# KrishnaswamyLab/MELD

Measured on AMD Instinct MI355X. Metric: cells/sec through MELD.fit_transform (kNN+Chebyshev), higher is better.
Workload: dtype f64

## Files before the change

### meld_amd/csrc/frame.hip

```cpp
#include "common.hpp"

namespace meld {

constexpr int FR_ROWS = 64;
constexpr int FR_DMAX = 64;

__global__ __launch_bounds__(256) void cov_sample_kernel(const double* __restrict__ X, int64_t n_s, int64_t stride, int d,
                                                         const double* __restrict__ mean, double* __restrict__ out) {
  __shared__ double sx[FR_ROWS][FR_DMAX + 1];
  const int tid = threadIdx.x;
  const int64_t s0 = (int64_t)blockIdx.x * FR_ROWS;
  const int cnt = (int)min((int64_t)FR_ROWS, n_s - s0);
  for (int u = tid; u < FR_ROWS * d; u += 256) {
    const int r = u / d, k = u - r * d;
    sx[r][k] = r < cnt ? X[(s0 + r) * stride * d + k] - mean[k] : 0.0;
  }
  __syncthreads();
  for (int p = tid; p < d * d; p += 256) {
    const int i = p / d, j = p - i * d;
    if (j < i) continue;
    double acc = 0.0;
    for (int r = 0; r < FR_ROWS; ++r) acc = fma(sx[r][i], sx[r][j], acc);
    atomicAdd(out + p, acc);
  }
}

typedef double f64x8 __attribute__((ext_vector_type(8)));
typedef const __attribute__((address_space(4))) f64x8* const_f64x8_ptr;
constexpr int FR_LD = FR_DMAX + 1;
constexpr int FR_NQ = FR_ROWS * FR_DMAX / 256;
constexpr int FR_CPG = FR_DMAX / 4;
__global__ __launch_bounds__(256) void rotate_rows_kernel(const double* __restrict__ X, int64_t N, int d, const double* __restrict__ mean,
                                                          const double* __restrict__ At, double* __restrict__ out, int64_t tiles_per_wg) {
  __shared__ double sx[FR_ROWS][FR_LD];
  const int tid = threadIdx.x, lane = tid & 63;
  const int w = __builtin_amdgcn_readfirstlane(tid >> 6);
  const int cpg = (d + 3) >> 2;
  const int j0 = w * cpg;
  const int k8n = (d + 7) >> 3;
  const double mk = (lane < d) ? mean[lane] : 0.0;
  const int64_t n_tiles = (N + FR_ROWS - 1) / FR_ROWS;
  const int64_t t_begin = (int64_t)blockIdx.x * tiles_per_wg, t_end = min(n_tiles, t_begin + tiles_per_wg);
  double xv[FR_NQ];
  auto fetch = [&](int64_t t) __attribute__((always_inline)) {
    const int64_t row0 = t * FR_ROWS;
#pragma unroll
    for (int q = 0; q < FR_NQ; ++q) {
      const int u = tid + 256 * q, rr = u >> 6, k = u & 63;
      xv[q] = (t < t_end && row0 + rr < N && k < d) ? X[(row0 + rr) * d + k] : mk;
    }
  };
  fetch(t_begin);
  for (int64_t t = t_begin; t < t_end; ++t) {
    const int64_t row0 = t * FR_ROWS;
    const int cnt = (int)min((int64_t)FR_ROWS, N - row0);
    __syncthreads();
#pragma unroll
    for (int q = 0; q < FR_NQ; ++q) {
      const int u = tid + 256 * q, rr = u >> 6, k = u & 63;
      sx[rr][k] = xv[q] - mk;
    }
    fetch(t + 1);
    __syncthreads();
    double xr[FR_DMAX];
#pragma unroll
    for (int k = 0; k < FR_DMAX; ++k) xr[k] = sx[lane][k];
    double res[FR_CPG];
#pragma unroll
    for (int c4 = 0; c4 < FR_CPG; c4 += 4) {
      double acc[4] = {0.0, 0.0, 0.0, 0.0};
      if (c4 < cpg) {
        const_f64x8_ptr arow[4];
#pragma unroll
        for (int i = 0; i < 4; ++i)
          arow[i] = (const_f64x8_ptr)(uintptr_t)(At + (size_t)min(j0 + c4 + i, d - 1) * FR_DMAX);
#pragma unroll
        for (int k8 = 0; k8 < FR_DMAX / 8; ++k8) {
          if (k8 < k8n) {
            f64x8 av[4];
#pragma unroll
            for (int i = 0; i < 4; ++i) av[i] = arow[i][k8];
#pragma unroll
            for (int e = 0; e < 8; ++e)
#pragma unroll
              for (int i = 0; i < 4; ++i) acc[i] = fma(xr[8 * k8 + e], av[i][e], acc[i]);
          }
        }
      }
#pragma unroll
      for (int i = 0; i < 4; ++i) res[c4 + i] = acc[i];
    }
    __syncthreads();
#pragma unroll
    for (int c = 0; c < FR_CPG; ++c)
      if (c < cpg && j0 + c < d) sx[lane][j0 + c] = res[c];
    __syncthreads();
#pragma unroll
    for (int q = 0; q < FR_NQ; ++q) {
      const int u = tid + 256 * q, rr = u >> 6, k = u & 63;
      if (rr < cnt && k < d) out[(row0 + rr) * d + k] = sx[rr][k];
    }
  }
}

}

using namespace meld;

extern "C" int meld_frame_max_dims(void) { return FR_DMAX; }

extern "C" int meld_cov_sample_f64(const double* X, int64_t N, int d, const double* mean, int64_t stride, double* cov, meld_stream_t stream) {
  MELD_CHECK_ARG(X && mean && cov && N > 0 && d > 0 && d <= FR_DMAX && stride >= 1, "meld_cov_sample_f64: bad arguments (d <= %d)", FR_DMAX);
  const int64_t n_s = (N + stride - 1) / stride;
  hipLaunchKernelGGL(cov_sample_kernel, dim3((unsigned)ceil_div(n_s, FR_ROWS)), dim3(256), 0, S(stream), X, n_s, stride, d, mean, cov);
  MELD_LAUNCH_CHECK("cov_sample_kernel");
  return MELD_OK;
}

extern "C" int meld_rotate_rows_f64(const double* X, int64_t N, int d, const double* mean, const double* At, double* out, meld_stream_t stream) {
  MELD_CHECK_ARG(X && mean && At && out && N > 0 && d > 0 && d <= FR_DMAX && X != out, "meld_rotate_rows_f64: bad arguments (d <= %d)", FR_DMAX);
  const int64_t tiles = ceil_div(N, FR_ROWS);
  const int64_t per = ceil_div(tiles, (int64_t)1024);
  hipLaunchKernelGGL(rotate_rows_kernel, dim3((unsigned)ceil_div(tiles, per)), dim3(256), 0, S(stream), X, N, d, mean, At, out, per);
  MELD_LAUNCH_CHECK("rotate_rows_kernel");
  return MELD_OK;
}
```

Before: 28.52 million.

## Rework rotate_rows kernel with templated column count, LDS-staged At and 2-row register tiling

The row-rotation kernel becomes a template on columns-per-wave, specialised at runtime from d. The At matrix and the mean are staged in dynamic LDS, each lane computes two rows per tile, the tile grows to 128 rows, and global loads and stores use contiguous flat indexing with a d-dependent padded LDS stride. The aim is to cut wasted work for d<64, reduce scalar global reads of At, and coalesce I/O. In exchange it adds sixteen instantiations, larger LDS use, and a hipFuncSetAttribute path. That path's size formula differs from the launch size, and the d&7 branch adds dummy fma no-ops.

New measurement: 28.44 million. About the same (-0.3%).

```diff
diff --git a/meld_amd/csrc/frame.hip b/meld_amd/csrc/frame.hip
--- a/meld_amd/csrc/frame.hip
+++ b/meld_amd/csrc/frame.hip
@@ -25,82 +25,105 @@
   }
 }
 
-typedef double f64x8 __attribute__((ext_vector_type(8)));
-typedef const __attribute__((address_space(4))) f64x8* const_f64x8_ptr;
-constexpr int FR_LD = FR_DMAX + 1;
-constexpr int FR_NQ = FR_ROWS * FR_DMAX / 256;
-constexpr int FR_CPG = FR_DMAX / 4;
-__global__ __launch_bounds__(256) void rotate_rows_kernel(const double* __restrict__ X, int64_t N, int d, const double* __restrict__ mean,
-                                                          const double* __restrict__ At, double* __restrict__ out, int64_t tiles_per_wg) {
-  __shared__ double sx[FR_ROWS][FR_LD];
+constexpr int RT_ROWS = 128;
+__host__ __device__ inline int rt_ld(int d) { return d + ((2 - d) & 3); }
+template <int C>
+__global__ __launch_bounds__(256, C <= 13 ? 2 : 1) void rotate_rows_kernel(const double* __restrict__ X, int64_t N, int d, const double* __restrict__ mean,
+                                                             const double* __restrict__ At, double* __restrict__ out, int64_t tiles_per_wg) {
+  extern __shared__ __attribute__((aligned(16))) double rt_lds[];
+  constexpr int NQ = 2 * C;
   const int tid = threadIdx.x, lane = tid & 63;
   const int w = __builtin_amdgcn_readfirstlane(tid >> 6);
-  const int cpg = (d + 3) >> 2;
-  const int j0 = w * cpg;
-  const int k8n = (d + 7) >> 3;
-  const double mk = (lane < d) ? mean[lane] : 0.0;
-  const int64_t n_tiles = (N + FR_ROWS - 1) / FR_ROWS;
+  const int ld = rt_ld(d), np = (d + 1) >> 1;
+  double* sx = rt_lds;
+  double* sa = sx + RT_ROWS * ld;
+  double* sm = sa + np * 4 * C * 2;
+  for (int u = tid; u < np * 4 * C * 2; u += 256) {
+    const int e = u & 1, j = (u >> 1) % (4 * C), k = 2 * ((u >> 1) / (4 * C)) + e;
+    sa[u] = (j < d && k < FR_DMAX) ? At[(size_t)j * FR_DMAX + k] : 0.0;
+  }
+  if (tid < d) sm[tid] = mean[tid];
+  for (int u = tid; u < RT_ROWS * (ld - d); u += 256) sx[(u / (ld - d)) * ld + d + u % (ld - d)] = 0.0;
+  const int r0 = tid / d, k0 = tid - r0 * d, dr = 256 / d, dk = 256 - dr * d;
+  const int64_t n_tiles = (N + RT_ROWS - 1) / RT_ROWS;
   const int64_t t_begin = (int64_t)blockIdx.x * tiles_per_wg, t_end = min(n_tiles, t_begin + tiles_per_wg);
-  double xv[FR_NQ];
+  double xv[NQ];
   auto fetch = [&](int64_t t) __attribute__((always_inline)) {
-    const int64_t row0 = t * FR_ROWS;
+    const int64_t row0 = t * RT_ROWS;
+    if (t >= t_end) return;
+    const int last = (int)min((int64_t)RT_ROWS, N - row0) * d - 1;
+    const double* src = X + row0 * d;
 #pragma unroll
-    for (int q = 0; q < FR_NQ; ++q) {
-      const int u = tid + 256 * q, rr = u >> 6, k = u & 63;
-      xv[q] = (t < t_end && row0 + rr < N && k < d) ? X[(row0 + rr) * d + k] : mk;
-    }
+    for (int q = 0; q < NQ; ++q) xv[q] = src[min(tid + 256 * q, last)];
   };
   fetch(t_begin);
   for (int64_t t = t_begin; t < t_end; ++t) {
-    const int64_t row0 = t * FR_ROWS;
-    const int cnt = (int)min((int64_t)FR_ROWS, N - row0);
+    const int64_t row0 = t * RT_ROWS;
+    const int n_el = (int)min((int64_t)RT_ROWS, N - row0) * d;
     __syncthreads();
+    {
+      int r = r0, k = k0;
 #pragma unroll
-    for (int q = 0; q < FR_NQ; ++q) {
-      const int u = tid + 256 * q, rr = u >> 6, k = u & 63;
-      sx[rr][k] = xv[q] - mk;
+      for (int q = 0; q < NQ; ++q) {
+        if (tid + 256 * q < RT_ROWS * d) sx[r * ld + k] = xv[q] - sm[k];
+        r += dr, k += dk;
+        if (k >= d) k -= d, ++r;
+      }
     }
     fetch(t + 1);
     __syncthreads();
-    double xr[FR_DMAX];
+    double acc[2][C];
 #pragma unroll
-    for (int k = 0; k < FR_DMAX; ++k) xr[k] = sx[lane][k];
-    double res[FR_CPG];
+    for (int c = 0; c < C; ++c) acc[0][c] = acc[1][c] = 0.0;
+    {
+      const double2* xa = (const double2*)(sx + lane * ld);
+      const double2* xb = (const double2*)(sx + (lane + 64) * ld);
+      const double2* ap = (const double2*)sa + w * C;
+#pragma unroll 1
+      for (int p = 0; p < np; ++p, ap += 4 * C) {
+        const double2 a = xa[p], b = xb[p];
+        double2 av[C];
 #pragma unroll
-    for (int c4 = 0; c4 < FR_CPG; c4 += 4) {
-      double acc[4] = {0.0, 0.0, 0.0, 0.0};
-      if (c4 < cpg) {
-        const_f64x8_ptr arow[4];
+        for (int c = 0; c < C; ++c) av[c] = ap[c];
 #pragma unroll
-        for (int i = 0; i < 4; ++i)
-          arow[i] = (const_f64x8_ptr)(uintptr_t)(At + (size_t)min(j0 + c4 + i, d - 1) * FR_DMAX);
+        for (int c = 0; c < C; ++c) acc[0][c] = fma(a.x, av[c].x, acc[0][c]), acc[1][c] = fma(b.x, av[c].x, acc[1][c]);
 #pragma unroll
-        for (int k8 = 0; k8 < FR_DMAX / 8; ++k8) {
-          if (k8 < k8n) {
-            f64x8 av[4];
+        for (int c = 0; c < C; ++c) acc[0][c] = fma(a.y, av[c].y, acc[0][c]), acc[1][c] = fma(b.y, av[c].y, acc[1][c]);
+      }
+    }
+    if (d & 7) {
 #pragma unroll
-            for (int i = 0; i < 4; ++i) av[i] = arow[i][k8];
-#pragma unroll
-            for (int e = 0; e < 8; ++e)
-#pragma unroll
-              for (int i = 0; i < 4; ++i) acc[i] = fma(xr[8 * k8 + e], av[i][e], acc[i]);
-          }
-        }
-      }
-#pragma unroll
-      for (int i = 0; i < 4; ++i) res[c4 + i] = acc[i];
+      for (int c = 0; c < C; ++c) acc[0][c] = fma(0.0, 0.0, acc[0][c]), acc[1][c] = fma(0.0, 0.0, acc[1][c]);
     }
     __syncthreads();
 #pragma unroll
-    for (int c = 0; c < FR_CPG; ++c)
-      if (c < cpg && j0 + c < d) sx[lane][j0 + c] = res[c];
+    for (int c = 0; c < C; ++c)
+      if (w * C + c < d) sx[lane * ld + w * C + c] = acc[0][c], sx[(lane + 64) * ld + w * C + c] = acc[1][c];
     __syncthreads();
+    {
+      double* dst = out + row0 * d;
+      int r = r0, k = k0;
 #pragma unroll
-    for (int q = 0; q < FR_NQ; ++q) {
-      const int u = tid + 256 * q, rr = u >> 6, k = u & 63;
-      if (rr < cnt && k < d) out[(row0 + rr) * d + k] = sx[rr][k];
+      for (int q = 0; q < NQ; ++q) {
+        if (tid + 256 * q < n_el) dst[tid + 256 * q] = sx[r * ld + k];
+        r += dr, k += dk;
+        if (k >= d) k -= d, ++r;
+      }
     }
   }
+}
+
+template <int C>
+static int rotate_rows_launch(const double* X, int64_t N, int d, const double* mean, const double* At, double* out, hipStream_t st) {
+  const size_t lds = sizeof(double) * ((size_t)RT_ROWS * rt_ld(d) + (size_t)((d + 1) / 2) * 4 * C * 2 + FR_DMAX);
+  if (lds > 64 * 1024)
+    MELD_HIP_CALL(hipFuncSetAttribute(reinterpret_cast<const void*>(&rotate_rows_kernel<C>), hipFuncAttributeMaxDynamicSharedMemorySize,
+                                      (int)(sizeof(double) * ((size_t)RT_ROWS * rt_ld(4 * C) + (size_t)2 * C * 4 * C * 2 + FR_DMAX))));
+  const int64_t tiles = ceil_div(N, RT_ROWS);
+  const int64_t per = ceil_div(tiles, (int64_t)1024);
+  hipLaunchKernelGGL(rotate_rows_kernel<C>, dim3((unsigned)ceil_div(tiles, per)), dim3(256), lds, st, X, N, d, mean, At, out, per);
+  MELD_LAUNCH_CHECK("rotate_rows_kernel");
+  return MELD_OK;
 }
 
 }
@@ -119,9 +142,11 @@
 
 extern "C" int meld_rotate_rows_f64(const double* X, int64_t N, int d, const double* mean, const double* At, double* out, meld_stream_t stream) {
   MELD_CHECK_ARG(X && mean && At && out && N > 0 && d > 0 && d <= FR_DMAX && X != out, "meld_rotate_rows_f64: bad arguments (d <= %d)", FR_DMAX);
-  const int64_t tiles = ceil_div(N, FR_ROWS);
-  const int64_t per = ceil_div(tiles, (int64_t)1024);
-  hipLaunchKernelGGL(rotate_rows_kernel, dim3((unsigned)ceil_div(tiles, per)), dim3(256), 0, S(stream), X, N, d, mean, At, out, per);
-  MELD_LAUNCH_CHECK("rotate_rows_kernel");
+  switch ((d + 3) / 4) {
+#define MELD_RT_CASE(C) case C: return rotate_rows_launch<C>(X, N, d, mean, At, out, S(stream));
+    MELD_RT_CASE(1) MELD_RT_CASE(2) MELD_RT_CASE(3) MELD_RT_CASE(4) MELD_RT_CASE(5) MELD_RT_CASE(6) MELD_RT_CASE(7) MELD_RT_CASE(8)
+    MELD_RT_CASE(9) MELD_RT_CASE(10) MELD_RT_CASE(11) MELD_RT_CASE(12) MELD_RT_CASE(13) MELD_RT_CASE(14) MELD_RT_CASE(15) MELD_RT_CASE(16)
+#undef MELD_RT_CASE
+  }
   return MELD_OK;
 }
```
